# bobocode/lmono

Hardware: AMD Instinct MI355X
Metric: KITTI HDL-64 scans/sec (scanRegistration + laserOdometry) (higher is better)
Workload: dtype f32 features / f64 solve

## Files before the change

### lmono_amd/csrc/lidar_abi.hip

```cpp
#pragma once
constexpr int kListGrid = 256;

struct lmono_scan_batch {
    lmono_ctx *ctx = nullptr;
    int n_cap = 0;
    int64_t pts_cap = 0;
    int n_scans = 0;
    int64_t total = 0;
    int max_pts = 0;
    bool registered = false;
    bool grid_built = false;
    std::vector<int64_t> off_h;
    bool validation_pending = false;
    DevOwner mem;
    BatchView v{};
    int64_t *off_d = nullptr;
    float *in_owned = nullptr;
    hipEvent_t staged_ev = nullptr, in_free_ev = nullptr;
    int64_t staged_points = -1;
    std::vector<int> feat_h;
    int chains_cap = 0;
    double *state = nullptr, *incr = nullptr, *poses = nullptr, *xq = nullptr;
    int *corr = nullptr, *lm_info = nullptr, *corr_pair = nullptr, *seed = nullptr;
    float4 *crec = nullptr, *crec_pair = nullptr;
    unsigned int *wl = nullptr;
    size_t wl_cap = 0;
    double *ws = nullptr, *resid_d = nullptr;
    int *rstat = nullptr;
    unsigned int *rcount = nullptr;
    hipEvent_t rep_ev[2] = { nullptr, nullptr };
    lmono_boundary_report brep{};
    std::vector<double> resid_h;
    std::vector<int> rerun_h;
    int last_chains = 0, last_lead = 0, last_first = 0;
};

extern "C" void lmono_batch_destroy(lmono_scan_batch *b)
{
    if (!b) return;
    b->mem.clear();
    for (auto &e : b->rep_ev) if (e) (void)hipEventDestroy(e);
    if (b->staged_ev) (void)hipEventDestroy(b->staged_ev);
    if (b->in_free_ev) (void)hipEventDestroy(b->in_free_ev);
    delete b;
}

extern "C" lmono_scan_batch *lmono_batch_create(lmono_ctx *c, int n_cap, int64_t pts_cap)
{
    if (!c || n_cap <= 0 || pts_cap <= 0) return nullptr;
    if (hipSetDevice(c->device) != hipSuccess) return nullptr;
    lmono_scan_batch *b = new lmono_scan_batch();
    b->ctx = c; b->n_cap = n_cap; b->pts_cap = pts_cap;
    BatchView &v = b->v;
    const size_t T = (size_t)pts_cap, N = (size_t)n_cap;
    DevOwner &m = b->mem;
    bool ok = true;
    ok = ok && m.alloc(b->off_d, N + 1);
    ok = ok && m.alloc(v.cloud, T) && m.alloc(v.curv, T) && m.alloc(v.label, T) && m.alloc(v.gap, T);
    ok = ok && m.alloc(v.ring_tmp, T);
    ok = ok && m.alloc(v.seg_hist, ((T >> 10) + N + 1) * 64) && m.alloc(v.scan_ends, N * 2) && m.alloc(v.scan_half, N) && m.alloc(v.scan_ori, N * 2);
    ok = ok && m.alloc(v.ring_begin, N * 65) && m.alloc(v.n_cloud, N) && m.alloc(v.status, N);
    ok = ok && m.alloc(v.sel_sharp, N * 64 * 6 * 20) && m.alloc(v.sel_sharp_n, N * 64 * 6);
    ok = ok && m.alloc(v.sel_flat, N * 64 * 6 * 4) && m.alloc(v.sel_flat_n, N * 64 * 6);
    ok = ok && m.alloc(v.lf_tmp, T) && m.alloc(v.lf_n, N * 64) && m.alloc(v.vox_todo, N * 64 + 1) && m.alloc(v.sel_todo, N * 64 + 1) && m.alloc(v.li_todo, N * 2 + 1);
    ok = ok && m.alloc(v.sharp, N * kMaxSharp) && m.alloc(v.less_sharp, N * kMaxLessSharp);
    ok = ok && m.alloc(v.flat, N * kMaxFlat) && m.alloc(v.less_flat, T);
    ok = ok && m.alloc(v.feat_n, N * 4) && m.alloc(v.line_first_ge, N * 2 * 66) && m.alloc(v.line_last_le, N * 2 * 66);
    ok = ok && m.alloc(v.cg_cell, N * kCornerTable) && m.alloc(v.sg_cell, N * kSurfTable);
    ok = ok && m.alloc(v.cg_pts, N * kMaxLessSharp) && m.alloc(v.sg_pts, T) && m.alloc(v.grid_mask, N * 2);
    ok = ok && m.alloc(v.lbc_pts, N * kMaxLessSharp + kLbPad) && m.alloc(v.lbs_pts, T + kLbPad) && m.alloc(v.lb_start, N * 2 * (kLineKeys + 1)) && m.alloc(v.lb_elev, N * 2 * 66);
    ok = ok && m.alloc(b->incr, N * 7) && m.alloc(b->poses, N * 7) && m.alloc(b->xq, 8);
    ok = ok && m.alloc(b->corr_pair, (size_t)kMaxQueries * 4) && m.alloc(b->crec_pair, (size_t)kMaxQueries * 4);
    if (!ok) {
        c->err = "lmono_batch_create: hipMalloc failed";
        lmono_batch_destroy(b);
        return nullptr;
    }
// ... 184 lines not shown
    if (!c || !b || !counts_h || !b->registered) return LMONO_EINVAL;
    const int n = b->n_scans;
    std::vector<int> nc(n), fn(n * 4), stt(n);
    HIP_TRY(c, hipStreamSynchronize(c->stream));
    HIP_TRY(c, hipMemcpy(nc.data(), b->v.n_cloud, sizeof(int) * n, hipMemcpyDeviceToHost));
    HIP_TRY(c, hipMemcpy(fn.data(), b->v.feat_n, sizeof(int) * n * 4, hipMemcpyDeviceToHost));
    HIP_TRY(c, hipMemcpy(stt.data(), b->v.status, sizeof(int) * n, hipMemcpyDeviceToHost));
    for (int s = 0; s < n; s++) {
        counts_h[6 * s] = nc[s];
        for (int k = 0; k < 4; k++) counts_h[6 * s + 1 + k] = fn[4 * s + k];
        counts_h[6 * s + 5] = stt[s];
    }
    return LMONO_OK;
}

extern "C" int lmono_batch_get_cloud(lmono_ctx *c, lmono_scan_batch *b, int scan, int which, float *out_h, int cap)
{
    if (!c || !b || !out_h || !b->registered || scan < 0 || scan >= b->n_scans || which < 0 || which > 4) return LMONO_EINVAL;
    HIP_TRY(c, hipStreamSynchronize(c->stream));
    int n = 0;
    const float4 *src = nullptr;
    int fn[4];
    HIP_TRY(c, hipMemcpy(fn, b->v.feat_n + scan * 4, sizeof(fn), hipMemcpyDeviceToHost));
    switch (which) {
    case 0: HIP_TRY(c, hipMemcpy(&n, b->v.n_cloud + scan, sizeof(int), hipMemcpyDeviceToHost)); src = b->v.cloud + b->off_h[scan]; break;
    case 1: n = fn[0]; src = b->v.sharp + (size_t)scan * kMaxSharp; break;
    case 2: n = fn[1]; src = b->v.less_sharp + (size_t)scan * kMaxLessSharp; break;
    case 3: n = fn[2]; src = b->v.flat + (size_t)scan * kMaxFlat; break;
    default: n = fn[3]; src = b->v.less_flat + b->off_h[scan]; break;
    }
    if (n > cap) { c->err = "get_cloud: output capacity too small"; return LMONO_ECAPACITY; }
    if (n > 0) HIP_TRY(c, hipMemcpy(out_h, src, sizeof(float4) * n, hipMemcpyDeviceToHost));
    return n;
}

extern "C" int lmono_batch_get_curvature(lmono_ctx *c, lmono_scan_batch *b, int scan, float *curv_h, int32_t *label_h, int cap)
{
    if (!c || !b || !b->registered || scan < 0 || scan >= b->n_scans) return LMONO_EINVAL;
    HIP_TRY(c, hipStreamSynchronize(c->stream));
    int n = 0;
    HIP_TRY(c, hipMemcpy(&n, b->v.n_cloud + scan, sizeof(int), hipMemcpyDeviceToHost));
    if (n > cap) { c->err = "get_curvature: output capacity too small"; return LMONO_ECAPACITY; }
    if (curv_h && n > 0) HIP_TRY(c, hipMemcpy(curv_h, b->v.curv + b->off_h[scan], sizeof(float) * n, hipMemcpyDeviceToHost));
    if (label_h && n > 0) {
        std::vector<int8_t> tmp(n);
        HIP_TRY(c, hipMemcpy(tmp.data(), b->v.label + b->off_h[scan], n, hipMemcpyDeviceToHost));
        for (int i = 0; i < n; i++) label_h[i] = tmp[i];
    }
    return n;
}

static int ensure_odom_ws(lmono_ctx *c, lmono_scan_batch *b, int n_chains)
{
    if (n_chains <= b->chains_cap) return LMONO_OK;
    DevOwner &m = b->mem;
    bool ok = m.alloc(b->state, (size_t)n_chains * 8) && m.alloc(b->corr, (size_t)n_chains * kMaxQueries * 4) &&
              m.alloc(b->lm_info, (size_t)n_chains * 4) && m.alloc(b->crec, (size_t)n_chains * kMaxQueries * 4) &&
              m.alloc(b->seed, (size_t)n_chains * kMaxQueries) && m.alloc(b->wl, 8 * ((size_t)n_chains * kMaxQueries + 1)) &&
              m.alloc(b->ws, (size_t)n_chains * 8) && m.alloc(b->resid_d, (size_t)n_chains) && m.alloc(b->rstat, (size_t)n_chains * 4) &&
              m.alloc(b->rcount, (size_t)n_chains + 2);
    if (!ok) { c->err = "odometry workspace: hipMalloc failed"; return LMONO_ENOMEM; }
    b->chains_cap = n_chains;
    return LMONO_OK;
}

static int ensure_grid(lmono_ctx *c, lmono_scan_batch *b)
{
    if (b->grid_built) return LMONO_OK;
#ifdef LMONO_DIAG_SEARCH
    hipLaunchKernelGGL(k_grid_build, dim3(b->n_scans, 1 + kGridPar), dim3(1024), kGridLds, c->stream, b->v);
    int rc = check_launch(c, "k_grid_build");
    if (rc) return rc;
    b->grid_built = true; b->v.has_grid = 1;
    return LMONO_OK;
#else
    c->err = "the hash-grid searches exist in the diagnostic build only (-DLMONO_DIAG_SEARCH)";
    return LMONO_EINVAL;
#endif
}

struct GroupFork {
    lmono_ctx *c; int G, g_own; bool forked = false;
    GroupFork(lmono_ctx *c_, int G_, int g_own_) : c(c_), G(G_), g_own(g_own_) {}
    int fork()
    {
        if (G <= 1) return LMONO_OK;
        for (int g = g_own; g < G; g++)
            if (!c->gstream[g]) {
                int lo = 0, hi = 0;
                if (c->odom_prio && hipDeviceGetStreamPriorityRange(&lo, &hi) == hipSuccess) HIP_TRY(c, hipStreamCreateWithPriority(&c->gstream[g], hipStreamNonBlocking, hi));
                else HIP_TRY(c, hipStreamCreateWithFlags(&c->gstream[g], hipStreamNonBlocking));
            }
        for (int g = 0; g <= G && g < 9; g++) if (!c->gev[g]) HIP_TRY(c, hipEventCreateWithFlags(&c->gev[g], hipEventDisableTiming));
        HIP_TRY(c, hipEventRecord(c->gev[0], c->stream));
        forked = true;
        for (int g = g_own; g < G; g++) HIP_TRY(c, hipStreamWaitEvent(c->gstream[g], c->gev[0], 0));
        return LMONO_OK;
    }
    int join()
    {
        if (!forked) return LMONO_OK;
        forked = false;
        int rc = LMONO_OK;
        for (int g = g_own; g < G; g++) {
            if (hipEventRecord(c->gev[g + 1], c->gstream[g]) != hipSuccess || hipStreamWaitEvent(c->stream, c->gev[g + 1], 0) != hipSuccess) {
                (void)hipStreamSynchronize(c->gstream[g]);
                c->err = "odometry: joining a chain-group stream failed"; rc = LMONO_ENODEV;
            }
        }
        return rc;
    }
    ~GroupFork() { (void)join(); }
};

static int odom_groups(const lmono_ctx *c, int n_ch)
{
    constexpr int kMinChainsPerGroup = 32;
    int G = c->opt[LMONO_OPT_ODOM_STREAMS];
    G = G < 1 ? 1 : (G > 8 ? 8 : G);
    if (c->stream != nullptr && G > 3 && !c->many_queues) G = 3;
    while (G > 1 && n_ch / G < kMinChainsPerGroup) G--;
    if (c->opt[LMONO_OPT_CORR_TILE] != 3) G = 1;
    return G;
}

static int odom_launch_steps(lmono_ctx *c, lmono_scan_batch *b, const OdomView &o, int n_ch, int step_a, int step_b, int G, EvSet *es, int *ne)
{
    const int tile = c->opt[LMONO_OPT_CORR_TILE];
    hipStream_t st = c->stream;
    const int g_own = st == nullptr ? 1 : 0;
    const size_t wl_stride = (size_t)b->chains_cap * kMaxQueries + 1;
    auto kev = [&](int i) -> hipEvent_t {
        if (!es) return nullptr;
        while ((int)es->kev.size() <= i) { hipEvent_t e; if (hipEventCreate(&e) != hipSuccess) return nullptr; es->kev.push_back(e); }
        return es->kev[i];
    };
    GroupFork fork(c, G, g_own);
    int rc = fork.fork();
    if (rc) return rc;
    for (int step = step_a; step < step_b; step++) {
        for (int outer = 0; outer < 2; outer++) {
            for (int g = 0; g < G; g++) {
                hipStream_t sg = (G == 1 || g < g_own) ? st : c->gstream[g];
                OdomView og = o;
                og.chain0 = (int)((long long)g * n_ch / G); og.chain1 = (int)((long long)(g + 1) * n_ch / G);
                const int ng = og.chain1 - og.chain0;
                if (ng <= 0) continue;
                unsigned int *wlg = b->wl + g * wl_stride;
                hipEvent_t e0 = nullptr, e1 = nullptr, e2 = nullptr;
                if (g == 0 && es) { e0 = kev(*ne); e1 = kev(*ne + 1); e2 = kev(*ne + 2); }
                if (e0 && e1 && e2) (void)hipEventRecord(e0, sg);
                if (tile == 3) {
                    hipLaunchKernelGGL(k_corr_flat, dim3(8 * ((ng + 7) / 8) * kCfBlocks), dim3(kCfT), 0, sg, b->v, og, step, outer, wlg, c->opt[LMONO_OPT_DEFER_EVERY], c->stats_d);
                    hipLaunchKernelGGL(k_correspond_list, dim3(kListGrid), dim3(256), 0, sg, b->v, og, step, outer, (const unsigned int *)wlg, c->stats_d);
                }
#ifdef LMONO_DIAG_SEARCH
                else
                    hipLaunchKernelGGL(k_correspond, dim3(8 * ((ng + 7) / 8) * kCorrBlocks), dim3(256), 0, sg, b->v, og, step, outer);
#endif
                if (e0 && e1 && e2) (void)hipEventRecord(e1, sg);
                hipLaunchKernelGGL(k_lm_solve, dim3(ng), dim3(kLmT), kLmRecLds, sg, b->v, og, step, outer, tile ? wlg : (unsigned int *)nullptr);
                if (e0 && e1 && e2) { (void)hipEventRecord(e2, sg); *ne += 3; }
            }
        }
    }
    return fork.join();
}

static int odom_validate(lmono_ctx *c, lmono_scan_batch *b, OdomView o, bool ext, bool first_call, EvSet *es = nullptr, int *ne = nullptr)
{
    hipStream_t st = c->stream;
    const int n_chains = o.n_chains;
    lmono_boundary_report &R = b->brep;
    if (first_call) {
        R = lmono_boundary_report{};
        R.n_chains = n_chains; R.tol = o.tol;
        b->resid_h.assign(n_chains, 0.0); b->rerun_h.assign(n_chains, 0);
    }
    if (!b->rep_ev[0]) for (auto &e : b->rep_ev) HIP_TRY(c, hipEventCreate(&e));
    HIP_TRY(c, hipEventRecord(b->rep_ev[0], st));
    int max_len = 0;
    for (int ch = 0; ch < n_chains; ch++) { int s, e; chain_bounds(o.first, o.n_scans, n_chains, ch, s, e); max_len = e - s > max_len ? e - s : max_len; }
    const int tile = c->opt[LMONO_OPT_CORR_TILE];
    std::vector<int> rs((size_t)n_chains * 4);
    const int max_rounds = n_chains + 1;
    int still_flagged = 0;
    for (int round = 0; round <= max_rounds; round++) {
        const bool very_first = first_call && round == 0;
        hipLaunchKernelGGL(k_boundary_check, dim3(1), dim3(256), 0, st, o, very_first ? b->resid_d : (double *)nullptr, very_first ? 1 : 0, ext ? 1 : 0);
        unsigned int cnt[2] = { 0, 0 };
        HIP_TRY(c, hipMemcpyAsync(cnt, b->rcount, sizeof(cnt), hipMemcpyDeviceToHost, st));
        if (very_first) HIP_TRY(c, hipMemcpyAsync(b->resid_h.data(), b->resid_d, sizeof(double) * n_chains, hipMemcpyDeviceToHost, st));
        HIP_TRY(c, hipStreamSynchronize(st));
        if (very_first) {
            for (int ch = 0; ch < n_chains; ch++) R.max_resid = b->resid_h[ch] > R.max_resid ? b->resid_h[ch] : R.max_resid;
            if (R.max_resid >= 1e299) { c->err = "odometry: a chain boundary holds a NaN increment (a scan pair without a usable solution)"; return LMONO_ESCAN; }
        }
        const int nf = (int)cnt[0];
        still_flagged = nf;
        if (nf == 0 || round == max_rounds) break;
        R.flagged += nf; R.rounds += 1;
        OdomView orp = o;
        orp.repair = 1; orp.clist = (const int *)(b->rcount + 2); orp.lead_full = -1;
        const int G = odom_groups(c, nf);
        if (tile) for (int g = 0; g < G; g++) HIP_TRY(c, hipMemsetAsync(b->wl + g * ((size_t)b->chains_cap * kMaxQueries + 1), 0, sizeof(unsigned int), st));
        int done = 0, chunk = 3;
        while (done < max_len) {
            const int upto = done + chunk < max_len ? done + chunk : max_len;
            orp.step0 = 0;
            int rc = odom_launch_steps(c, b, orp, nf, done, upto, G, es, ne);
            if (rc) return rc;
            done = upto;
            HIP_TRY(c, hipMemcpyAsync(cnt, b->rcount, sizeof(cnt), hipMemcpyDeviceToHost, st));
            HIP_TRY(c, hipStreamSynchronize(st));
            if (cnt[1] == 0) break;
            chunk = chunk < 8 ? chunk * 2 : 8;
        }
    }
    HIP_TRY(c, hipEventRecord(b->rep_ev[1], st));
    HIP_TRY(c, hipMemcpyAsync(rs.data(), b->rstat, sizeof(int) * 4 * n_chains, hipMemcpyDeviceToHost, st));
    HIP_TRY(c, hipStreamSynchronize(st));
    float ms = 0.f;
    if (hipEventElapsedTime(&ms, b->rep_ev[0], b->rep_ev[1]) == hipSuccess) R.repair_ms += ms;
    R.pairs_rerun = 0; R.chains_rerun = 0;
    R.unresolved = still_flagged;
    for (int ch = 0; ch < n_chains; ch++) {
        b->rerun_h[ch] = rs[ch * 4 + 1];
        R.pairs_rerun += rs[ch * 4 + 1]; R.chains_rerun += rs[ch * 4 + 3] > 0 ? 1 : 0;
    }
    return check_launch(c, "boundary validation");
}

static OdomView odom_view(lmono_ctx *c, lmono_scan_batch *b, int n_chains, int lead, int first)
{
    OdomView o{};
    o.n_scans = b->n_scans; o.n_chains = n_chains; o.lead = lead; o.first = first; o.fixed_k = -1; o.chain0 = 0; o.chain1 = n_chains;
    o.lead_full = c->opt[LMONO_OPT_CORR_TILE] == 3 ? c->opt[LMONO_OPT_LEAD_FULL] : -1;
    o.state = b->state; o.corr = b->corr; o.incr = b->incr; o.lm_info = b->lm_info; o.crec = b->crec; o.seed = b->seed;
    o.ws = b->ws; o.repair = 0; o.step0 = 0; o.clist = nullptr; o.rstat = b->rstat; o.rcount = b->rcount;
    o.tol = 1e-9 * (double)c->opt[LMONO_OPT_BOUNDARY_TOL];
    return o;
}

static int odom_run(lmono_ctx *c, lmono_scan_batch *b, int n_chains, int lead, int first, double *incr_d, double *poses_d, bool want_poses, bool validate = true)
{
    if (!c || !b || !b->registered || lead < 0 || first < 0 || first >= b->n_scans) return LMONO_EINVAL;
    const int n = b->n_scans;
    if (n_chains < 1) n_chains = 1;
    if (n_chains > n - first) n_chains = n - first;
    HIP_TRY(c, hipSetDevice(c->device));
    int rc = ensure_odom_ws(c, b, n_chains);
    if (rc) return rc;
    OdomView o = odom_view(c, b, n_chains, lead, first);
    b->last_chains = n_chains; b->last_lead = lead; b->last_first = first;
    int max_steps = 0;
    for (int ch = 0; ch < n_chains; ch++) {
        int s, e;
        chain_bounds(first, n, n_chains, ch, s, e);
        const int begin = s - lead > 0 ? s - lead : 0;
        const int steps = e - begin - 1;
        max_steps = steps > max_steps ? steps : max_steps;
    }
    hipStream_t st = c->stream;
    if (c->n_sets == 0 || c->sets[c->n_sets - 1].odom) c->ev = c->next_set();
    if (!c->ev) { c->err = "hipEventCreate failed"; return LMONO_ENODEV; }
    c->sets[c->n_sets - 1].odom = true;
    HIP_TRY(c, hipEventRecord(c->ev[8], st));
    const int ninit = n > n_chains ? n : n_chains;
    hipLaunchKernelGGL(k_odom_init, dim3((ninit + 255) / 256), dim3(256), 0, st, o);
    const int tile = c->opt[LMONO_OPT_CORR_TILE];
    if (tile != 3) { rc = ensure_grid(c, b); if (rc) return rc; }
    const int G = odom_groups(c, n_chains);
    if (tile) for (int g = 0; g < G; g++) HIP_TRY(c, hipMemsetAsync(b->wl + g * ((size_t)b->chains_cap * kMaxQueries + 1), 0, sizeof(unsigned int), st));
    EvSet &es = c->sets[c->n_sets - 1];
    int ne = 0;
    if (c->opt[LMONO_OPT_LEAD_SEED] > 0 && n_chains > 2 && lead >= 3 && max_steps > 1 && o.ws) {
        rc = odom_launch_steps(c, b, o, n_chains, 0, 1, G, &es, &ne);
        if (rc) return rc;
        hipLaunchKernelGGL(k_lead_seed_median, dim3((n_chains + 255) / 256), dim3(256), 0, st, o);
        hipLaunchKernelGGL(k_lead_seed_apply, dim3((n_chains + 255) / 256), dim3(256), 0, st, o);
        rc = odom_launch_steps(c, b, o, n_chains, 1, max_steps, G, &es, &ne);
    } else
        rc = odom_launch_steps(c, b, o, n_chains, 0, max_steps, G, &es, &ne);
    if (rc) return rc;
    es.n_kev = ne;
    b->brep = lmono_boundary_report{};
    b->brep.n_chains = n_chains;
    b->resid_h.assign((size_t)n_chains, 0.0); b->rerun_h.assign((size_t)n_chains, 0);
    b->validation_pending = !validate;
    if (validate && o.tol > 0.0 && n_chains > 1) { rc = odom_validate(c, b, o, false, true); if (rc) return rc; }
    if (want_poses) hipLaunchKernelGGL(k_pose_prefix, dim3(1), dim3(64), 0, st, (const double *)b->incr, b->poses, first, n);
// ... 250 lines not shown
```

### lmono_amd/csrc/lmono_hip.hip

```cpp
#include "line_index.hip"
#include "frontend.hip"
#include "trust_region.hpp"
#include "odometry.hip"
#include "corr_flat.hip"
#include "mapping.hip"
#include "ba.hip"
#include "ba_solve.hip"
#include "feat.hip"
#include "marg.hip"

#include <string>
#include <vector>
#include <thread>
#include <mutex>
#include <condition_variable>
#include <atomic>
#include <functional>
#include <memory>
#include <chrono>
#include <algorithm>
#include <cstdio>
#include <cstring>


using namespace lmono;

struct EvSet { hipEvent_t e[10]; bool reg = false, odom = false; std::vector<hipEvent_t> kev; int n_kev = 0; };

#include "host_workers.hpp"
#include "dev_owner.hpp"

struct MapPlanScratch {
    struct Run { int ind, at, len; };
    std::vector<char> is_valid; std::vector<int> add, fill, cand; std::vector<int64_t> cat_off; std::vector<Run> runs;
    MapPlanScratch() : is_valid((size_t)lmono::kMdCubes, 0), add((size_t)lmono::kMdCubes, 0), fill((size_t)lmono::kMdCubes, 0), cat_off((size_t)lmono::kMdCubes, -1) {}
};

struct lmono_ctx {
    int device = 0;
    hipStream_t stream = nullptr;
    std::string err;
    std::vector<EvSet> sets;
    int n_sets = 0;
    hipEvent_t *ev = nullptr;
    int opt[LMONO_OPT_COUNT] = { 3, 0, 4, -1, 1000, 0, 0 };
    hipStream_t gstream[8] = { nullptr, nullptr, nullptr, nullptr, nullptr, nullptr, nullptr, nullptr };
    hipEvent_t gev[9] = { nullptr, nullptr, nullptr, nullptr, nullptr, nullptr, nullptr, nullptr, nullptr };
    unsigned long long *stats_d = nullptr;
    hipStream_t copy_stream = nullptr;
    hipStream_t own_stream = nullptr;
    bool odom_prio = false, many_queues = false;
    struct Chunk { char *base; size_t cap; };
    std::vector<Chunk> arena;
    size_t arena_chunk = 0, arena_off = 0;
    int n_cu = 0;
    int map_budget = 0;
    int cluster_budget = 0;
    char *stage = nullptr;
    size_t stage_cap = 0;
    std::vector<void *> stage_all;
    std::vector<MapPlanScratch> plan_scratch;
    std::unique_ptr<HostWorkers> workers;

    hipEvent_t *next_set()
    {
        constexpr int kMaxSets = 1024;
        if (n_sets == (int)sets.size()) {
            if (n_sets >= kMaxSets) { sets[n_sets - 1].reg = sets[n_sets - 1].odom = false; return sets[n_sets - 1].e; }
            EvSet s;
            for (auto &e : s.e) if (hipEventCreate(&e) != hipSuccess) return nullptr;
            sets.push_back(s);
        }
        sets[n_sets].reg = sets[n_sets].odom = false;
        sets[n_sets].n_kev = 0;
        return sets[n_sets++].e;
    }
};

#define HIP_TRY(ctx, expr)                                                                   \
    do {                                                                                     \
        hipError_t e_ = (expr);                                                              \
        if (e_ != hipSuccess) {                                                              \
            (ctx)->err = std::string(#expr) + ": " + hipGetErrorString(e_);                  \
            return e_ == hipErrorOutOfMemory ? LMONO_ENOMEM : LMONO_ENODEV;                  \
        }                                                                                    \
    } while (0)

static int check_launch(lmono_ctx *c, const char *what)
{
    hipError_t e = hipGetLastError();
    if (e != hipSuccess) { c->err = std::string(what) + ": " + hipGetErrorString(e); return LMONO_ENODEV; }
    return LMONO_OK;
}

namespace {
struct DevBuf {
    lmono_ctx *c;
    size_t chunk0, off0;
    bool used = false;
    static constexpr size_t kStageMax = (size_t)256 << 10;
    char *run_dst = nullptr;
    size_t run_at = 0, run_bytes = 0, stage_used = 0;
    explicit DevBuf(lmono_ctx *c_) : c(c_), chunk0(c_ ? c_->arena_chunk : 0), off0(c_ ? c_->arena_off : 0) {}
    bool send_run()
// ... 36 lines not shown
    template <typename T> T *up(const T *src, size_t n, bool &ok)
    {
        if (!ok || !c) { ok = false; return nullptr; }
        used = true;
        const size_t bytes = (((n > 0 ? n : 1) * sizeof(T)) + 255) & ~(size_t)255;
        while (c->arena_chunk < c->arena.size() && c->arena_off + bytes > c->arena[c->arena_chunk].cap) { c->arena_chunk++; c->arena_off = 0; }
        if (c->arena_chunk == c->arena.size()) {
            size_t cap = c->arena.empty() ? (size_t)1 << 20 : 2 * c->arena.back().cap;
            while (cap < bytes) cap <<= 1;
            void *q = nullptr;
            if (hipMalloc(&q, cap) != hipSuccess) { ok = false; return nullptr; }
            c->arena.push_back({ (char *)q, cap });
            c->arena_off = 0;
        }
        char *q = c->arena[c->arena_chunk].base + c->arena_off;
        c->arena_off += bytes;
        if (!src || n == 0) { if (!send_run()) ok = false; return (T *)q; }
        if (bytes > kStageMax) {
            if (!send_run() || hipMemcpyAsync(q, src, n * sizeof(T), hipMemcpyHostToDevice, c->stream) != hipSuccess) ok = false;
            return (T *)q;
        }
        if (stage_used + bytes > c->stage_cap) {
            if (!send_run()) ok = false;
            size_t cap = c->stage_cap ? 2 * c->stage_cap : (size_t)4 << 20;
            while (cap < bytes) cap <<= 1;
            void *h = nullptr;
            if (hipHostMalloc(&h, cap, hipHostMallocDefault) != hipSuccess) { ok = false; return nullptr; }
            c->stage_all.push_back(h); c->stage = (char *)h; c->stage_cap = cap; stage_used = 0;
        }
        if (run_bytes > 0 && q != run_dst + run_bytes) { if (!send_run()) ok = false; }
        if (run_bytes == 0) { run_dst = q; run_at = stage_used; }
        memcpy(c->stage + stage_used, src, n * sizeof(T));
        stage_used += bytes; run_bytes += bytes;
        return (T *)q;
    }
};
}

#ifdef LMONO_DIAG_SEARCH
extern "C" const char *lmono_version(void) { return "lmono-hip 0.4 (gfx950, diagnostic build: + hash-grid search)"; }
#else
extern "C" const char *lmono_version(void) { return "lmono-hip 0.4 (gfx950)"; }
#endif

extern "C" lmono_ctx *lmono_create(int device)
{
    int n = 0;
    if (hipGetDeviceCount(&n) != hipSuccess || n <= 0 || device < 0 || device >= n) return nullptr;
    if (hipSetDevice(device) != hipSuccess) return nullptr;
    lmono_ctx *c = new lmono_ctx();
    c->device = device;
    if (const char *e = getenv("LMONO_ODOM_STREAM_PRIORITY")) c->odom_prio = atoi(e) != 0;
    if (const char *e = getenv("GPU_MAX_HW_QUEUES")) c->many_queues = atoi(e) >= 8;
    {
        hipDeviceProp_t prop;
        if (hipGetDeviceProperties(&prop, device) != hipSuccess) { delete c; return nullptr; }
        c->n_cu = prop.multiProcessorCount;
        int per_cu = 0;
        if (hipOccupancyMaxActiveBlocksPerMultiprocessor(&per_cu, (const void *)k_ba_solve<true, false>, kBaT, 0) != hipSuccess || per_cu < 1) per_cu = 1;
        c->cluster_budget = std::max(8, c->n_cu * per_cu / 2);
        c->map_budget = std::max(8, c->n_cu / 2);
        if (const char *e = getenv("LMONO_CLUSTER_BUDGET")) { const int v = atoi(e); if (v >= 1) c->cluster_budget = c->map_budget = v; }
    }
    if (hipMalloc((void **)&c->stats_d, 320) != hipSuccess || hipMemset(c->stats_d, 0, 320) != hipSuccess) { delete c; return nullptr; }
    if (hipFuncSetAttribute((const void *)k_select, hipFuncAttributeMaxDynamicSharedMemorySize, 4 * sel_slice_bytes(kRingCap) + 4 * kSelScratch) != hipSuccess) { delete c; return nullptr; }
    if (hipFuncSetAttribute((const void *)k_voxel<kVoxSmallSlots, kVoxSmallBits, true>, hipFuncAttributeMaxDynamicSharedMemorySize, kVoxLdsSmall) != hipSuccess) { delete c; return nullptr; }
    if (hipFuncSetAttribute((const void *)k_voxel<kVoxBigSlots, kVoxBigBits, false>, hipFuncAttributeMaxDynamicSharedMemorySize, kVoxLdsBig) != hipSuccess) { delete c; return nullptr; }
    if (hipFuncSetAttribute((const void *)k_lm_solve, hipFuncAttributeMaxDynamicSharedMemorySize, kLmRecLds) != hipSuccess) { delete c; return nullptr; }
#ifdef LMONO_DIAG_SEARCH
    if (hipFuncSetAttribute((const void *)k_grid_build, hipFuncAttributeMaxDynamicSharedMemorySize, kGridLds) != hipSuccess) { delete c; return nullptr; }
#endif
    if (hipFuncSetAttribute((const void *)k_compact_index, hipFuncAttributeMaxDynamicSharedMemorySize, kLiLdsHalf) != hipSuccess) { delete c; return nullptr; }
    if (hipFuncSetAttribute((const void *)k_line_index<false>, hipFuncAttributeMaxDynamicSharedMemorySize, kLiLdsFull) != hipSuccess) { delete c; return nullptr; }
    if (hipFuncSetAttribute((const void *)k_marginalize, hipFuncAttributeMaxDynamicSharedMemorySize, (int)sizeof(MargLds)) != hipSuccess) { delete c; return nullptr; }
    if (hipFuncSetAttribute((const void *)k_marg_second_new, hipFuncAttributeMaxDynamicSharedMemorySize, (int)sizeof(Marg2Lds)) != hipSuccess) { delete c; return nullptr; }
#ifdef LMONO_TILE_PROF
    {
        int nb = 0;
        (void)hipOccupancyMaxActiveBlocksPerMultiprocessor(&nb, (const void *)k_corr_flat, kCfT, 0);
        std::fprintf(stderr, "[lmono diag] k_corr_flat: %d workgroups of %d threads per CU by the occupancy query, static LDS %zu B\n", nb, kCfT, sizeof(CfLds));
        (void)hipOccupancyMaxActiveBlocksPerMultiprocessor(&nb, (const void *)k_compact_index, kLiT, kLiLdsHalf);
        std::fprintf(stderr, "[lmono diag] k_compact_index: %d workgroups of %d threads per CU by the occupancy query, dynamic LDS %d B\n", nb, kLiT, kLiLdsHalf);
    }
#endif
    return c;
}

extern "C" void lmono_destroy(lmono_ctx *c)
{
    if (!c) return;
#ifdef LMONO_BOUNDS
    {
        unsigned long long o[4] = { 0, 0, 0, 0 };
        (void)hipDeviceSynchronize();
        if (hipMemcpyFromSymbol(o, HIP_SYMBOL(g_ba_oob), sizeof(o)) == hipSuccess)
            fprintf(stderr, "[lmono bounds] k_ba_solve: %llu access(es) outside the batch's allocation (first: ba_solve.hip:%llu, byte offset %lld, block %llu)\n", o[0], o[1], (long long)o[2], o[3]);
    }
#endif
    for (auto &s : c->sets) { for (auto &e : s.e) (void)hipEventDestroy(e); for (auto &e : s.kev) (void)hipEventDestroy(e); }
    if (c->stats_d) (void)hipFree(c->stats_d);
    for (auto &s : c->gstream) if (s) (void)hipStreamDestroy(s);
    if (c->copy_stream) (void)hipStreamDestroy(c->copy_stream);
    for (void *h : c->stage_all) (void)hipHostFree(h);
    if (c->own_stream) (void)hipStreamDestroy(c->own_stream);
    for (auto &ch : c->arena) (void)hipFree(ch.base);
    for (auto &e : c->gev) if (e) (void)hipEventDestroy(e);
    delete c;
}

extern "C" const char *lmono_last_error(const lmono_ctx *c) { return c ? c->err.c_str() : "null context"; }

extern "C" int lmono_set_stream(lmono_ctx *c, void *s)
{
    if (!c) return LMONO_EINVAL;
    c->stream = (hipStream_t)s;
    return LMONO_OK;
}

extern "C" int lmono_use_own_stream(lmono_ctx *c)
{
    if (!c) return LMONO_EINVAL;
// ... 70 lines not shown
```

### lmono_amd/csrc/odometry.hip

```cpp
#include "batch.hpp"

namespace lmono {

constexpr float kCell = 1.0f;
constexpr float kInvCell = 1.0f;
constexpr int kMaxShell = 6;
constexpr int kCoordOff = 1 << 20;
constexpr int kRunMaxCount = 32767;
__device__ __forceinline__ int pack_run(int start, int count) { return start | (count << 17); }

__device__ __forceinline__ unsigned long long cell_key(int cx, int cy, int cz)
{
    return ((unsigned long long)(unsigned int)(cx + kCoordOff) << 42) |
           ((unsigned long long)(unsigned int)(cy + kCoordOff) << 21) |
           (unsigned long long)(unsigned int)(cz + kCoordOff);
}
__device__ __forceinline__ unsigned int hash_key(unsigned long long k)
{
    const unsigned int cz = (unsigned int)(k & 0x1fffffull), cy = (unsigned int)((k >> 21) & 0x1fffffull), cx = (unsigned int)(k >> 42);
    unsigned int h = (cx * 73856093u) ^ (cy * 19349663u) ^ (cz * 83492791u);
    h ^= h >> 15;
    return h;
}

// ... 136 lines not shown
            if (pass == 0) {
                before = wave_sum_i(before);
                if (lane == 0 && before) atomicAdd(&s_before, before);
            }
            if (fail) s_fail = 1;
            __syncthreads();
            if (pass == 0) {
                const int per = P >> 10;
                int c[16], sum = 0;
                int occ = 0;
#pragma unroll
                for (int q = 0; q < 16; q++) { c[q] = q < per ? cnt[tid * per + q] : 0; sum += c[q]; occ += c[q] > 0 ? 1 : 0; }
                const int incl = wave_scan_incl(sum);
                if (lane == 63) s_wsum[wave] = incl;
                occ = wave_sum_i(occ);
                if (lane == 0 && occ) atomicAdd(&s_occ, occ);
                __syncthreads();
                if (s_occ >= P) s_fail = 1;
                int run = s_before + incl - sum;
                for (int w = 0; w < wave; w++) run += s_wsum[w];
#pragma unroll
                for (int q = 0; q < 16; q++) { if (q < per) { cnt[tid * per + q] = run; run += c[q]; } }
                __syncthreads();
            }
        }
        const bool bad = s_fail != 0;
        bool dense = false;
        for (int j = tid; j < P; j += 1024) {
            const unsigned int k = keys[j];
            const int end = cnt[j], start = j > 0 ? cnt[j - 1] : s_before;
            const int c = end - start;
            GridCell e;
            e.key = (k == kEmptyKey32 || bad) ? kEmptyKey : key32_to_64(k);
            e.cnt = bad ? 0 : c;
            e.start = bad ? 0 : start;
            cell[(size_t)p * P + j] = e;
            dense = dense || c > kRunMaxCount;
        }
        if (tid == 0 && bad) atomicOr(&b.status[s], kStatusGridOverflow);
        if (dense) atomicOr(&b.status[s], kStatusDenseCell);
        __syncthreads();
    }
}
#endif
struct OdomView {
    int n_scans, n_chains, lead;
    int first;
    int chain0, chain1;
    int fixed_k;
    int lead_full;
    double *state;
    int *corr;
    float4 *crec;
    double *incr;
    int *lm_info;
    int *seed;
    double *ws;
    int repair;
    int step0;
    const int *clist;
    int *rstat;
    unsigned int *rcount;
    double tol;
};

__device__ __host__ __forceinline__ void chain_bounds(int first, int n_scans, int n_chains, int c, int &s, int &e)
{
    s = first + (int)((long long)c * (n_scans - first) / n_chains);
    e = first + (int)((long long)(c + 1) * (n_scans - first) / n_chains);
}

__device__ __forceinline__ void quat_rotate(const double *q, double vx, double vy, double vz, double &ox, double &oy, double &oz)
{
    const double ux = q[0], uy = q[1], uz = q[2], w = q[3];
    const double uvx = 2.0 * (uy * vz - uz * vy);
    const double uvy = 2.0 * (uz * vx - ux * vz);
    const double uvz = 2.0 * (ux * vy - uy * vx);
    ox = vx + w * uvx + (uy * uvz - uz * uvy);
    oy = vy + w * uvy + (uz * uvx - ux * uvz);
    oz = vz + w * uvz + (ux * uvy - uy * uvx);
}

__device__ __forceinline__ unsigned long long wave_nn(const GridRef &g, float qx, float qy, float qz, int lane)
{
    const int cqx = (int)floorf(qx * kInvCell), cqy = (int)floorf(qy * kInvCell), cqz = (int)floorf(qz * kInvCell);
    unsigned long long best = ~0ull;
    for (int sh = 1; sh <= kMaxShell; sh++) {
        const int side = 2 * sh + 1, ncell = side * side * side;
        for (int base = 0; base < ncell; base += 64) {
            const int ci = base + lane;
            int st = 0, cn = 0;
            if (ci < ncell) {
                const int dx = ci % side - sh, dy = (ci / side) % side - sh, dz = ci / (side * side) - sh;
                if (sh == 1 || max(max(abs(dx), abs(dy)), abs(dz)) == sh) {
                    const unsigned long long k = cell_key(cqx + dx, cqy + dy, cqz + dz);
                    unsigned int sl = hash_key(k) & g.mask;
                    const unsigned int pmask = min((unsigned int)g.mask, (unsigned int)(kGridPage - 1));
                    while (true) {
                        const GridCell e = g.cell[sl];
                        if (e.key == k) { st = e.start; cn = e.cnt; break; }
                        if (e.key == kEmptyKey) break;
                        sl = grid_next(sl, pmask);
                    }
                }
            }
            unsigned long long m = __ballot(cn > 0);
// ... 514 lines not shown
{
    const int kind = __float_as_int(cp.w);
    if (kind == 1) {
        const double ex = (double)A.x - (double)B.x, ey = (double)A.y - (double)B.y, ez = (double)A.z - (double)B.z;
        const double inv = 1.0 / sqrt(ex * ex + ey * ey + ez * ez);
        P[0] = (double)A.x; P[1] = (double)A.y; P[2] = (double)A.z;
        P[3] = ex * inv; P[4] = ey * inv; P[5] = ez * inv;
    } else {
        const double jx = (double)A.x, jy = (double)A.y, jz = (double)A.z;
        const double ux = jx - (double)B.x, uy = jy - (double)B.y, uz = jz - (double)B.z;
        const double wx = jx - (double)Cc.x, wy = jy - (double)Cc.y, wz = jz - (double)Cc.z;
        double nx = uy * wz - uz * wy, ny = uz * wx - ux * wz, nz = ux * wy - uy * wx;
        const double nn = sqrt(nx * nx + ny * ny + nz * nz);
        if (nn > 0.0) { nx /= nn; ny /= nn; nz /= nn; }
        P[0] = jx; P[1] = jy; P[2] = jz; P[3] = nx; P[4] = ny; P[5] = nz;
    }
}

__device__ __forceinline__ void lm_row(LmAcc &acc, double d0, double d1, double d2, double rvx, double rvy, double rvz, double res, double sr)
{
#pragma clang fp contract(fast)
    double J[6];
    const double s2 = 2.0 * sr;
    J[0] = (rvy * d2 - rvz * d1) * s2; J[1] = (rvz * d0 - rvx * d2) * s2; J[2] = (rvx * d1 - rvy * d0) * s2;
    J[3] = d0 * sr; J[4] = d1 * sr; J[5] = d2 * sr;
    accumulate_row(acc, J, res * sr);
}

template <bool kJac, bool kEdge>
__device__ __forceinline__ void eval_block(const float4 cp, const double2 P01, const double2 P23, const double2 P45, const double *Rm, const double *x, LmAcc &acc)
{
#pragma clang fp contract(fast)
    if (__float_as_int(cp.w) == 0) return;
    const double vx = (double)cp.x, vy = (double)cp.y, vz = (double)cp.z;
    const double rvx = Rm[0] * vx + Rm[1] * vy + Rm[2] * vz, rvy = Rm[3] * vx + Rm[4] * vy + Rm[5] * vz, rvz = Rm[6] * vx + Rm[7] * vy + Rm[8] * vz;
    const double dx = rvx + x[4] - P01.x, dy = rvy + x[5] - P01.y, dz = rvz + x[6] - P23.x;
    const double qx = P23.y, qy = P45.x, qz = P45.y;
    double r0, r1 = 0.0, r2 = 0.0, sq;
    if (kEdge) { r0 = dy * qz - dz * qy; r1 = dz * qx - dx * qz; r2 = dx * qy - dy * qx; sq = r0 * r0 + r1 * r1 + r2 * r2; }
    else { r0 = dx * qx + dy * qy + dz * qz; sq = r0 * r0; }
    double rho0, rho1;
    huber(sq, rho0, rho1);
    acc.cost += 0.5 * rho0;
    if (!kJac) return;
    const double sr = rho1 == 1.0 ? 1.0 : sqrt(rho1);
    if (kEdge) {
        lm_row(acc, 0.0, qz, -qy, rvx, rvy, rvz, r0, sr);
        lm_row(acc, -qz, 0.0, qx, rvx, rvy, rvz, r1, sr);
        lm_row(acc, qy, -qx, 0.0, rvx, rvy, rvz, r2, sr);
    } else
        lm_row(acc, qx, qy, qz, rvx, rvy, rvz, r0, sr);
}

template <bool kJac>
__device__ __forceinline__ void evaluate_block(const float4 *srec, int n_edge, int nq, const double *x, double (*s_red)[28], double *s_sum)
{
    const int tid = threadIdx.x, lane = tid & 63, wave = tid >> 6;
    LmAcc acc;
    acc.cost = 0.0;
    if (kJac) {
#pragma unroll
        for (int i = 0; i < 21; i++) acc.H[i] = 0.0;
#pragma unroll
        for (int i = 0; i < 6; i++) acc.g[i] = 0.0;
    }
    double Rm[9];
    {
#pragma clang fp contract(fast)
        const double ux = x[0], uy = x[1], uz = x[2], w = x[3];
        Rm[0] = 1.0 - 2.0 * (uy * uy + uz * uz); Rm[1] = 2.0 * (ux * uy - w * uz);       Rm[2] = 2.0 * (ux * uz + w * uy);
        Rm[3] = 2.0 * (ux * uy + w * uz);       Rm[4] = 1.0 - 2.0 * (ux * ux + uz * uz); Rm[5] = 2.0 * (uy * uz - w * ux);
        Rm[6] = 2.0 * (ux * uz - w * uy);       Rm[7] = 2.0 * (uy * uz + w * ux);       Rm[8] = 1.0 - 2.0 * (ux * ux + uy * uy);
    }
    const double2 *sp = (const double2 *)srec;
    int qi = tid;
    for (; qi < n_edge; qi += kLmT)
        eval_block<kJac, true>(srec[qi], sp[kMaxQueries + qi], sp[2 * kMaxQueries + qi], sp[3 * kMaxQueries + qi], Rm, x, acc);
    for (; qi < nq; qi += kLmT)
        eval_block<kJac, false>(srec[qi], sp[kMaxQueries + qi], sp[2 * kMaxQueries + qi], sp[3 * kMaxQueries + qi], Rm, x, acc);
    acc.cost = wave_sum_d(acc.cost);
    if (kJac) {
#pragma unroll
        for (int i = 0; i < 21; i++) acc.H[i] = wave_sum_d(acc.H[i]);
#pragma unroll
        for (int i = 0; i < 6; i++) acc.g[i] = wave_sum_d(acc.g[i]);
    }
    __syncthreads();
    if (lane == 0) {
        s_red[wave][27] = acc.cost;
        if (kJac) {
            for (int i = 0; i < 21; i++) s_red[wave][i] = acc.H[i];
            for (int i = 0; i < 6; i++) s_red[wave][21 + i] = acc.g[i];
        }
    }
    __syncthreads();
    if (tid < 28 && (kJac || tid == 27)) {
        double t = 0.0;
        for (int w = 0; w < kLmW; w++) t += s_red[w][tid];
        s_sum[tid] = t;
    }
    __syncthreads();
}

constexpr int kLmRecLds = 4 * kMaxQueries * 16;
#ifndef LMONO_CF_T
#define LMONO_CF_T 128
#endif
constexpr int kThinBlocks = kMaxQueries / LMONO_CF_T;

#ifndef LMONO_LM_MAX_ITER
#define LMONO_LM_MAX_ITER 4
#endif

__global__ __launch_bounds__(kLmT) void k_lm_solve(BatchView b, OdomView o, int step, int outer, unsigned int *wl_reset)
{
    const int c = o.clist ? o.clist[o.chain0 + blockIdx.x] : o.chain0 + (int)blockIdx.x;
    if (wl_reset && blockIdx.x == 0 && threadIdx.x == 0) wl_reset[0] = 0u;
    int s;
    const int k = chain_scan(o, c, step, s);
    if (k < 0) return;
    __shared__ double s_red[kLmW][28], s_sum[28], s_cur[28];
    __shared__ int s_used[kLmW];
    const int tid = threadIdx.x, lane = tid & 63, wave = tid >> 6;
    const int n_edge = b.feat_n[k * 4 + 0], nq = n_edge + b.feat_n[k * 4 + 2];
    const float4 *crec = o.crec + (size_t)c * kMaxQueries * 4;
    extern __shared__ __align__(16) float4 s_rec[];
    int n_used = 0;
    {
        double2 *sp = (double2 *)s_rec;
        const bool thin = lead_in_thinned(o, k, s);
        for (int qi = tid; qi < nq; qi += kLmT) {
            float4 cp = crec[qi * 4];
            const float4 A = crec[qi * 4 + 1], B = crec[qi * 4 + 2], Cc = crec[qi * 4 + 3];
            if (thin && (qi % kThinBlocks) % kThinStride != 0) cp.w = 0.f;
            double P[6] = { 0.0, 0.0, 0.0, 0.0, 0.0, 0.0 };
            if (__float_as_int(cp.w) != 0) { stage_block(cp, A, B, Cc, P); n_used++; }
            s_rec[qi] = cp;
            sp[kMaxQueries + qi] = make_double2(P[0], P[1]);
            sp[2 * kMaxQueries + qi] = make_double2(P[2], P[3]);
            sp[3 * kMaxQueries + qi] = make_double2(P[4], P[5]);
        }
    }
    __syncthreads();
    double x[7];
    for (int i = 0; i < 7; i++) x[i] = o.state[c * 8 + i];

    evaluate_block<true>(s_rec, n_edge, nq, x, s_red, s_sum);
    n_used = wave_sum_i(n_used);
    if (lane == 0) s_used[wave] = n_used;
    __syncthreads();
    n_used = 0;
    for (int w = 0; w < kLmW; w++) n_used += s_used[w];
    TrustRegion<true> tr(LMONO_LM_MAX_ITER);
    auto take = [&]() {
        __syncthreads();
        if (tid < 28) s_cur[tid] = s_sum[tid];
        __syncthreads();
    };
    if (tid < 28) s_cur[tid] = s_sum[tid];
    __syncthreads();
    if (n_used > 0 && tr.begin(s_cur, x))
        for (;;) {
            double cand[7];
            if (tr.propose(s_cur, x, cand) == 2) break;
            if (tr.last()) evaluate_block<false>(s_rec, n_edge, nq, cand, s_red, s_sum);
            else evaluate_block<true>(s_rec, n_edge, nq, cand, s_red, s_sum);
            if (!tr.judge(s_sum, s_cur, x, cand, take)) break;
        }
    if (tid == 0) {
        for (int i = 0; i < 7; i++) o.state[c * 8 + i] = x[i];
        if (o.repair && outer == 1) {
            int e0, e1;
            chain_bounds(o.first, o.n_scans, o.n_chains, c, e0, e1);
            const double res = boundary_residual(x, o.incr + (size_t)k * 7);
            for (int i = 0; i < 7; i++) o.incr[(size_t)k * 7 + i] = x[i];
            o.rstat[c * 4 + 1] += 1;
            int agree = o.rstat[c * 4 + 2] >> 1;
            agree = res <= o.tol ? agree + 1 : 0;
            o.rstat[c * 4 + 2] = 1 | (agree << 1);
            if (agree >= kRepairAgree || k + 1 >= e1) { o.rstat[c * 4] = 1; atomicSub(&o.rcount[1], 1u); }
        } else if (o.incr && outer == 1 && k >= s)
            for (int i = 0; i < 7; i++) o.incr[(size_t)k * 7 + i] = x[i];
        if (o.ws && !o.repair && outer == 1 && k == s - 1)
            for (int i = 0; i < 7; i++) o.ws[c * 8 + i] = x[i];
        if (o.lm_info) { o.lm_info[c * 4 + outer] = tr.iter; o.lm_info[c * 4 + 2 + outer] = n_used; }
    }
}

__global__ __launch_bounds__(256) void k_boundary_check(OdomView o, double *resid, int first_round, int ext)
{
    __shared__ int s_n;
    if (threadIdx.x == 0) s_n = 0;
    __syncthreads();
    for (int base = 0; base < o.n_chains; base += 256) {
        const int c = base + threadIdx.x;
        bool flag = false;
        if (c < o.n_chains) {
            int s, e;
            chain_bounds(o.first, o.n_scans, o.n_chains, c, s, e);
            double res = 0.0;
            if ((c > 0 || ext) && s > 0) res = boundary_residual(o.ws + c * 8, o.incr + (size_t)(s - 1) * 7);
            if (resid) resid[c] = res;
            flag = res > o.tol;
            if (first_round) { o.rstat[c * 4 + 1] = 0; o.rstat[c * 4 + 3] = 0; }
            o.rstat[c * 4] = flag ? 0 : 1;
            o.rstat[c * 4 + 2] = flag ? 1 : 0;
            if (flag) {
                o.rstat[c * 4 + 3] += 1;
                for (int i = 0; i < 7; i++) { const double v = o.incr[(size_t)(s - 1) * 7 + i]; o.state[c * 8 + i] = v; o.ws[c * 8 + i] = v; }
            }
        }
        const unsigned long long m = __ballot(flag);
        __shared__ int s_w[4];
        if ((threadIdx.x & 63) == 0) s_w[threadIdx.x >> 6] = __popcll(m);
        __syncthreads();
        int pre = s_n;
        for (int w = 0; w < (int)(threadIdx.x >> 6); w++) pre += s_w[w];
        if (flag) o.rcount[2 + pre + __popcll(m & ((1ull << (threadIdx.x & 63)) - 1ull))] = (unsigned int)c;
        __syncthreads();
// ... 127 lines not shown
```

Measured before the change: 127,100.

## Move LM solve staging records from LDS to global memory with software prefetch

Result: faster. 128,800 (median of 6 runs) (+1.3%).

```diff
diff --git a/lmono_amd/csrc/lidar_abi.hip b/lmono_amd/csrc/lidar_abi.hip
--- a/lmono_amd/csrc/lidar_abi.hip
+++ b/lmono_amd/csrc/lidar_abi.hip
@@ -23,6 +23,8 @@
     double *state = nullptr, *incr = nullptr, *poses = nullptr, *xq = nullptr;
     int *corr = nullptr, *lm_info = nullptr, *corr_pair = nullptr, *seed = nullptr;
     float4 *crec = nullptr, *crec_pair = nullptr;
+    float4 *lmrec = nullptr;
+    size_t lmrec_cap = 0;
     unsigned int *wl = nullptr;
     size_t wl_cap = 0;
     double *ws = nullptr, *resid_d = nullptr;
@@ -313,8 +315,13 @@
 
 static int ensure_odom_ws(lmono_ctx *c, lmono_scan_batch *b, int n_chains)
 {
+    DevOwner &m = b->mem;
+    const size_t lmrec_need = (size_t)(n_chains > b->chains_cap ? n_chains : b->chains_cap) * (4 - c->lm_planes) * kMaxQueries;
+    if (lmrec_need > b->lmrec_cap) {
+        if (!m.alloc(b->lmrec, lmrec_need)) { c->err = "odometry workspace: hipMalloc failed"; return LMONO_ENOMEM; }
+        b->lmrec_cap = lmrec_need;
+    }
     if (n_chains <= b->chains_cap) return LMONO_OK;
-    DevOwner &m = b->mem;
     bool ok = m.alloc(b->state, (size_t)n_chains * 8) && m.alloc(b->corr, (size_t)n_chains * kMaxQueries * 4) &&
               m.alloc(b->lm_info, (size_t)n_chains * 4) && m.alloc(b->crec, (size_t)n_chains * kMaxQueries * 4) &&
               m.alloc(b->seed, (size_t)n_chains * kMaxQueries) && m.alloc(b->wl, 8 * ((size_t)n_chains * kMaxQueries + 1)) &&
@@ -420,7 +427,9 @@
                     hipLaunchKernelGGL(k_correspond, dim3(8 * ((ng + 7) / 8) * kCorrBlocks), dim3(256), 0, sg, b->v, og, step, outer);
 #endif
                 if (e0 && e1 && e2) (void)hipEventRecord(e1, sg);
-                hipLaunchKernelGGL(k_lm_solve, dim3(ng), dim3(kLmT), kLmRecLds, sg, b->v, og, step, outer, tile ? wlg : (unsigned int *)nullptr);
+                unsigned int *wlr = tile ? wlg : (unsigned int *)nullptr;
+                if (c->lm_planes == 4) hipLaunchKernelGGL(k_lm_solve<4>, dim3(ng), dim3(kLmT), lm_rec_lds(4), sg, b->v, og, step, outer, wlr);
+                else hipLaunchKernelGGL(k_lm_solve<0>, dim3(ng), dim3(kLmT), lm_rec_lds(0), sg, b->v, og, step, outer, wlr);
                 if (e0 && e1 && e2) { (void)hipEventRecord(e2, sg); *ne += 3; }
             }
         }
@@ -497,7 +506,7 @@
     OdomView o{};
     o.n_scans = b->n_scans; o.n_chains = n_chains; o.lead = lead; o.first = first; o.fixed_k = -1; o.chain0 = 0; o.chain1 = n_chains;
     o.lead_full = c->opt[LMONO_OPT_CORR_TILE] == 3 ? c->opt[LMONO_OPT_LEAD_FULL] : -1;
-    o.state = b->state; o.corr = b->corr; o.incr = b->incr; o.lm_info = b->lm_info; o.crec = b->crec; o.seed = b->seed;
+    o.state = b->state; o.corr = b->corr; o.incr = b->incr; o.lm_info = b->lm_info; o.crec = b->crec; o.lmrec = b->lmrec; o.seed = b->seed;
     o.ws = b->ws; o.repair = 0; o.step0 = 0; o.clist = nullptr; o.rstat = b->rstat; o.rcount = b->rcount;
     o.tol = 1e-9 * (double)c->opt[LMONO_OPT_BOUNDARY_TOL];
     return o;
diff --git a/lmono_amd/csrc/lmono_hip.hip b/lmono_amd/csrc/lmono_hip.hip
--- a/lmono_amd/csrc/lmono_hip.hip
+++ b/lmono_amd/csrc/lmono_hip.hip
@@ -50,6 +50,7 @@
     hipStream_t copy_stream = nullptr;
     hipStream_t own_stream = nullptr;
     bool odom_prio = false, many_queues = false;
+    int lm_planes = kLmPlanesDefault;
     struct Chunk { char *base; size_t cap; };
     std::vector<Chunk> arena;
     size_t arena_chunk = 0, arena_off = 0;
@@ -192,6 +193,7 @@
     c->device = device;
     if (const char *e = getenv("LMONO_ODOM_STREAM_PRIORITY")) c->odom_prio = atoi(e) != 0;
     if (const char *e = getenv("GPU_MAX_HW_QUEUES")) c->many_queues = atoi(e) >= 8;
+    if (const char *e = getenv("LMONO_LM_LDS_PLANES")) { const int v = atoi(e); if (lm_planes_valid(v)) c->lm_planes = v; }
     {
         hipDeviceProp_t prop;
         if (hipGetDeviceProperties(&prop, device) != hipSuccess) { delete c; return nullptr; }
@@ -206,7 +208,7 @@
     if (hipFuncSetAttribute((const void *)k_select, hipFuncAttributeMaxDynamicSharedMemorySize, 4 * sel_slice_bytes(kRingCap) + 4 * kSelScratch) != hipSuccess) { delete c; return nullptr; }
     if (hipFuncSetAttribute((const void *)k_voxel<kVoxSmallSlots, kVoxSmallBits, true>, hipFuncAttributeMaxDynamicSharedMemorySize, kVoxLdsSmall) != hipSuccess) { delete c; return nullptr; }
     if (hipFuncSetAttribute((const void *)k_voxel<kVoxBigSlots, kVoxBigBits, false>, hipFuncAttributeMaxDynamicSharedMemorySize, kVoxLdsBig) != hipSuccess) { delete c; return nullptr; }
-    if (hipFuncSetAttribute((const void *)k_lm_solve, hipFuncAttributeMaxDynamicSharedMemorySize, kLmRecLds) != hipSuccess) { delete c; return nullptr; }
+    if (hipFuncSetAttribute((const void *)k_lm_solve<4>, hipFuncAttributeMaxDynamicSharedMemorySize, lm_rec_lds(4)) != hipSuccess) { delete c; return nullptr; }
 #ifdef LMONO_DIAG_SEARCH
     if (hipFuncSetAttribute((const void *)k_grid_build, hipFuncAttributeMaxDynamicSharedMemorySize, kGridLds) != hipSuccess) { delete c; return nullptr; }
 #endif
diff --git a/lmono_amd/csrc/odometry.hip b/lmono_amd/csrc/odometry.hip
--- a/lmono_amd/csrc/odometry.hip
+++ b/lmono_amd/csrc/odometry.hip
@@ -212,6 +212,7 @@
     double *state;
     int *corr;
     float4 *crec;
+    float4 *lmrec;
     double *incr;
     int *lm_info;
     int *seed;
@@ -832,8 +833,38 @@
         lm_row(acc, qx, qy, qz, rvx, rvy, rvz, r0, sr);
 }
 
-template <bool kJac>
-__device__ __forceinline__ void evaluate_block(const float4 *srec, int n_edge, int nq, const double *x, double (*s_red)[28], double *s_sum)
+struct LmBlk { float4 cp; double2 p01, p23, p45; };
+template <int kPlanes>
+struct LmRec {
+    static_assert(kPlanes == 0 || kPlanes == 4, "the instantiations the library holds");
+    float4 *lds;
+    float4 *mem;
+    template <int p> __device__ __forceinline__ float4 *plane() const { return p < kPlanes ? lds + p * kMaxQueries : mem + (p - kPlanes) * kMaxQueries; }
+    __device__ __forceinline__ void put(int qi, const float4 cp, const double *P) const
+    {
+        plane<0>()[qi] = cp;
+        ((double2 *)plane<1>())[qi] = make_double2(P[0], P[1]);
+        ((double2 *)plane<2>())[qi] = make_double2(P[2], P[3]);
+        ((double2 *)plane<3>())[qi] = make_double2(P[4], P[5]);
+    }
+    __device__ __forceinline__ void request(int qi, LmBlk &k) const
+    {
+        if (kPlanes < 1) k.cp = plane<0>()[qi];
+        if (kPlanes < 2) k.p01 = ((const double2 *)plane<1>())[qi];
+        if (kPlanes < 3) k.p23 = ((const double2 *)plane<2>())[qi];
+        if (kPlanes < 4) k.p45 = ((const double2 *)plane<3>())[qi];
+    }
+    __device__ __forceinline__ void local(int qi, LmBlk &k) const
+    {
+        if (kPlanes >= 1) k.cp = plane<0>()[qi];
+        if (kPlanes >= 2) k.p01 = ((const double2 *)plane<1>())[qi];
+        if (kPlanes >= 3) k.p23 = ((const double2 *)plane<2>())[qi];
+        if (kPlanes >= 4) k.p45 = ((const double2 *)plane<3>())[qi];
+    }
+};
+
+template <bool kJac, int kPlanes>
+__device__ __forceinline__ void evaluate_block(const LmRec<kPlanes> rec, int n_edge, int nq, const double *x, double (*s_red)[28], double *s_sum)
 {
     const int tid = threadIdx.x, lane = tid & 63, wave = tid >> 6;
     LmAcc acc;
@@ -852,12 +883,32 @@
         Rm[3] = 2.0 * (ux * uy + w * uz);       Rm[4] = 1.0 - 2.0 * (ux * ux + uz * uz); Rm[5] = 2.0 * (uy * uz - w * ux);
         Rm[6] = 2.0 * (ux * uz - w * uy);       Rm[7] = 2.0 * (uy * uz + w * ux);       Rm[8] = 1.0 - 2.0 * (ux * ux + uy * uy);
     }
-    const double2 *sp = (const double2 *)srec;
     int qi = tid;
-    for (; qi < n_edge; qi += kLmT)
-        eval_block<kJac, true>(srec[qi], sp[kMaxQueries + qi], sp[2 * kMaxQueries + qi], sp[3 * kMaxQueries + qi], Rm, x, acc);
-    for (; qi < nq; qi += kLmT)
-        eval_block<kJac, false>(srec[qi], sp[kMaxQueries + qi], sp[2 * kMaxQueries + qi], sp[3 * kMaxQueries + qi], Rm, x, acc);
+    if (kPlanes == 4) {
+        const float4 *srec = rec.lds;
+        const double2 *sp = (const double2 *)srec;
+        for (; qi < n_edge; qi += kLmT)
+            eval_block<kJac, true>(srec[qi], sp[kMaxQueries + qi], sp[2 * kMaxQueries + qi], sp[3 * kMaxQueries + qi], Rm, x, acc);
+        for (; qi < nq; qi += kLmT)
+            eval_block<kJac, false>(srec[qi], sp[kMaxQueries + qi], sp[2 * kMaxQueries + qi], sp[3 * kMaxQueries + qi], Rm, x, acc);
+    } else {
+        LmBlk cur = {}, nxt;
+        if (qi < nq) rec.request(qi, cur);
+        for (; qi < n_edge; qi += kLmT) {
+            nxt = cur;
+            if (qi + kLmT < nq) rec.request(qi + kLmT, nxt);
+            rec.local(qi, cur);
+            eval_block<kJac, true>(cur.cp, cur.p01, cur.p23, cur.p45, Rm, x, acc);
+            cur = nxt;
+        }
+        for (; qi < nq; qi += kLmT) {
+            nxt = cur;
+            if (qi + kLmT < nq) rec.request(qi + kLmT, nxt);
+            rec.local(qi, cur);
+            eval_block<kJac, false>(cur.cp, cur.p01, cur.p23, cur.p45, Rm, x, acc);
+            cur = nxt;
+        }
+    }
     acc.cost = wave_sum_d(acc.cost);
     if (kJac) {
 #pragma unroll
@@ -882,7 +933,12 @@
     __syncthreads();
 }
 
-constexpr int kLmRecLds = 4 * kMaxQueries * 16;
+constexpr int lm_rec_lds(int planes) { return planes * kMaxQueries * 16; }
+constexpr int kLmPlanesDefault = 0;
+__host__ inline bool lm_planes_valid(int planes) { return planes == 4 || planes == 0; }
+#ifndef LMONO_LM_VGPRS
+#define LMONO_LM_VGPRS 240
+#endif
 #ifndef LMONO_CF_T
 #define LMONO_CF_T 128
 #endif
@@ -892,7 +948,8 @@
 #define LMONO_LM_MAX_ITER 4
 #endif
 
-__global__ __launch_bounds__(kLmT) void k_lm_solve(BatchView b, OdomView o, int step, int outer, unsigned int *wl_reset)
+template <int kPlanes>
+__global__ __launch_bounds__(kLmT) __attribute__((amdgpu_num_vgpr(LMONO_LM_VGPRS / 2))) void k_lm_solve(BatchView b, OdomView o, int step, int outer, unsigned int *wl_reset)
 {
     const int c = o.clist ? o.clist[o.chain0 + blockIdx.x] : o.chain0 + (int)blockIdx.x;
     if (wl_reset && blockIdx.x == 0 && threadIdx.x == 0) wl_reset[0] = 0u;
@@ -905,9 +962,9 @@
     const int n_edge = b.feat_n[k * 4 + 0], nq = n_edge + b.feat_n[k * 4 + 2];
     const float4 *crec = o.crec + (size_t)c * kMaxQueries * 4;
     extern __shared__ __align__(16) float4 s_rec[];
+    const LmRec<kPlanes> rec = { s_rec, kPlanes < 4 ? o.lmrec + (size_t)c * (4 - kPlanes) * kMaxQueries : nullptr };
     int n_used = 0;
     {
-        double2 *sp = (double2 *)s_rec;
         const bool thin = lead_in_thinned(o, k, s);
         for (int qi = tid; qi < nq; qi += kLmT) {
             float4 cp = crec[qi * 4];
@@ -915,17 +972,14 @@
             if (thin && (qi % kThinBlocks) % kThinStride != 0) cp.w = 0.f;
             double P[6] = { 0.0, 0.0, 0.0, 0.0, 0.0, 0.0 };
             if (__float_as_int(cp.w) != 0) { stage_block(cp, A, B, Cc, P); n_used++; }
-            s_rec[qi] = cp;
-            sp[kMaxQueries + qi] = make_double2(P[0], P[1]);
-            sp[2 * kMaxQueries + qi] = make_double2(P[2], P[3]);
-            sp[3 * kMaxQueries + qi] = make_double2(P[4], P[5]);
+            rec.put(qi, cp, P);
         }
     }
     __syncthreads();
     double x[7];
     for (int i = 0; i < 7; i++) x[i] = o.state[c * 8 + i];
 
-    evaluate_block<true>(s_rec, n_edge, nq, x, s_red, s_sum);
+    evaluate_block<true>(rec, n_edge, nq, x, s_red, s_sum);
     n_used = wave_sum_i(n_used);
     if (lane == 0) s_used[wave] = n_used;
     __syncthreads();
@@ -943,8 +997,8 @@
         for (;;) {
             double cand[7];
             if (tr.propose(s_cur, x, cand) == 2) break;
-            if (tr.last()) evaluate_block<false>(s_rec, n_edge, nq, cand, s_red, s_sum);
-            else evaluate_block<true>(s_rec, n_edge, nq, cand, s_red, s_sum);
+            if (tr.last()) evaluate_block<false>(rec, n_edge, nq, cand, s_red, s_sum);
+            else evaluate_block<true>(rec, n_edge, nq, cand, s_red, s_sum);
             if (!tr.judge(s_sum, s_cur, x, cand, take)) break;
         }
     if (tid == 0) {
```
